# bladesaber/or-tools

Hardware: AMD Instinct MI355X
Metric: simplex iterations/sec + batched LPs/sec, 1/2/4/8 MI355X vs Glop CPU (higher is better)
Workload: dtype f64

## Files before the change

include/mi_lp_devop.h:

```cpp
#ifndef MI_LP_DEVOP_H_
#define MI_LP_DEVOP_H_

#include <stdint.h>

#ifdef __cplusplus
extern "C" {
#endif

typedef struct mi_devop mi_devop;

enum {
  MI_DEVOP_ROW_NONE = 0,
  MI_DEVOP_ROW_SMALL_SERIAL = 1,
  MI_DEVOP_ROW_SMALL_SERIAL_256 = 2,
  MI_DEVOP_ROW_SMALL_BY_COLUMN = 3,
  MI_DEVOP_ROW_MEDIUM_DIRECT = 4,
  MI_DEVOP_ROW_MEDIUM_BATCHED = 5,
  MI_DEVOP_ROW_LIST = 6,
  MI_DEVOP_ROW_FULL_ROWS = 7,
  MI_DEVOP_ROW_CHUNK = 8,
  MI_DEVOP_ROW_BY_COLUMN = 9,
  MI_DEVOP_ROW_COLUMN_WISE_SMALL = 10,
  MI_DEVOP_ROW_COLUMN_WISE_GENERAL = 11
};
enum { MI_DEVOP_COMPACT_NONE = 0, MI_DEVOP_COMPACT_SMALL = 1, MI_DEVOP_COMPACT_CHIP_WIDE = 2 };
enum { MI_DEVOP_RATIO_NONE = 0, MI_DEVOP_RATIO_ONE_WORKGROUP = 1, MI_DEVOP_RATIO_TWO_KERNELS = 2 };

typedef struct mi_devop_paths {
  int32_t update_row;
  int32_t compact;
  int32_t ratio;
  int32_t ratio_tightened;
  int32_t list_mapped;
} mi_devop_paths;

typedef struct mi_devop_api {
  mi_devop* (*create)(int device, int m, int n, const int64_t* col_starts,
                      const int32_t* row_idx, const double* vals);
  void (*destroy)(mi_devop* h);
  const char* (*last_error)(const mi_devop* h);
  int (*set_mask)(mi_devop* h, int which, const uint64_t* words, int num_words);
// ... 6 lines not shown
  int (*read_coefficient)(mi_devop* h, int col, double* out);
  int (*download_coefficients)(mi_devop* h, double* out);
  int (*list_dots_over_update_row)(mi_devop* h, const double* v, double* out, int* count);
  int (*list_dots)(mi_devop* h, const int32_t* cols, int n, const double* v, double* out);
  int (*dual_begin)(mi_devop* h, const double* rc, const uint8_t* colbits,
                    const double* bound_diff);
  int (*dual_set_col_bits)(mi_devop* h, const int32_t* cols, const uint8_t* bits, int n);
  int (*dual_ratio_candidates)(mi_devop* h, double sign, double threshold,
                               double harris_tolerance, double minimum_delta,
                               double variation_magnitude, int32_t* col, double* coeff,
                               double* rc, int* count, int* list_count);
  int (*dual_update_reduced_costs)(mi_devop* h, double mult, int leaving_col,
                                   double leaving_value, int entering_col);
  int (*dual_download_reduced_costs)(mi_devop* h, double* rc);
  int (*last_paths)(mi_devop* h, mi_devop_paths* out);
} mi_devop_api;

extern const mi_devop_api mi_devop_table;

#ifdef __cplusplus
}
#endif

#endif
```

or-tools_amd/csrc/engine/device_lp.h:

```cpp
#ifndef MILP_DEVICE_LP_H_
#define MILP_DEVICE_LP_H_

#include <cstdint>
#include <memory>
#include <mutex>
#include <stdexcept>
#include <string>
#include <vector>

#include "../../../include/mi_lp.h"
#include "device_solver.h"

namespace milp_kernels {
struct TriSolveArgs;
struct ScanState;
struct ListOut;
struct TightenState;
}
namespace sdual {
struct Mailbox;
}

namespace milp {
void SdualProfileReset();
// ... 117 lines not shown
    std::vector<int> runs;
    int chain_levels = 0;
    int max_wide_run = 0;
    int level0_end = 0;
  };
  struct TriContext {
    void* stream = nullptr;
    TriBuffer x, y, top;
    double* h_x = nullptr;
    double* m_x = nullptr;
    size_t h_x_elems = 0;
    int* h_top = nullptr;
    void* graph_exec[kTriNumMatrices] = {};
    uint64_t graph_key[kTriNumMatrices] = {};
    void* ev[2] = {nullptr, nullptr};
  };
  bool TransposeLowerSolve(const TriangularMatrix& t, uint64_t key,
                           std::vector<double>* x) override;
  bool LowerSolve(const TriangularMatrix& lower, uint64_t key,
                  std::vector<double>* x) override;
  bool Solve(TriKind kind, const TriangularMatrix& t, uint64_t key, int start,
             std::vector<double>* x) override;
  bool SolvePair(TriKind kind, const TriangularMatrix& t, uint64_t key, std::vector<double>* x0,
                 std::vector<double>* x1) override;
  bool StartAsyncU(const TriangularMatrix& t, uint64_t key, const std::vector<double>& x) override;
  void FinishAsyncU(std::vector<double>* x) override;
  void DropAsyncU() override;
  bool SpecFlipEnabled() const { return spec_flip_ && tri_mapped_ && !tri_graph_; }

  void SetTiming(bool on, uint32_t id_mask = ~0u);
  bool Timed(int id) const { return timing_ && (timing_ids_ >> (id & 31) & 1u) != 0; }
// ... 118 lines not shown
  void LaunchColumnDots(int mode, const double* d_y, const double* d_c, double* d_out,
                        const double* d_y2 = nullptr, double* d_out2 = nullptr);
  void Check(int err, const char* what);
  void BuildTriSchedule(TriSchedule* s, int nc, int fni, bool ones, const double* diag,
                        const int64_t* st, const int32_t* idx, const double* val, bool reverse,
                        bool descending, bool sequential, uint64_t key, void* stream);
  bool TriSolve(int which, const TriangularMatrix& t, uint64_t key, std::vector<double>* x);
  bool TriPrepare(int which, const TriangularMatrix& t, uint64_t key, int slot,
                  const std::vector<double>& x);
  void TransposeColumns(const TriangularMatrix& t, bool descending);
  void TriReserve(TriBuffer* b, size_t bytes);
  void PrepareTriContext(int slot, int rows, int pos);
  milp_kernels::TriSolveArgs TriArgs(const TriSchedule& s, const TriContext& c) const;
  void TriCopyIn(const TriSchedule& s, const TriContext& c);
  void TriCopyOut(const TriSchedule& s, const TriContext& c);
  void EnqueueTriKernels(const TriSchedule& s, const milp_kernels::TriSolveArgs& a,
                         void* stream);
  void CaptureTriGraph(int which, TriContext* c);
  void FreeTriBuffers();

  void* sdual_arena_ = nullptr;
  void* sdual_staging_ = nullptr;
  void* sdual_staging_dev_ = nullptr;
  size_t sdual_cap_ = 0;
  void* sdual_mb_block_ = nullptr;
  size_t sdual_mb_cap_ = 0;
  sdual::Mailbox* sdual_mb_ = nullptr;
  int32_t* sdual_mb_basis_ = nullptr;
  char* sdual_mb_image_ = nullptr;
  void* sdual_mb_device_ = nullptr;

  int device_ = -1;
// ... 184 lines not shown
  unsigned long long* d_keys_in_ = nullptr;
  unsigned long long* d_keys_out_ = nullptr;
  int32_t* d_sorted_slots_ = nullptr;
  void* d_sort_temp_ = nullptr;
  size_t sort_temp_bytes_ = 0;
  int tri_mode_ = 0;
  int tri_min_rows_ = 16384;
  int tri_wide_level_ = 600;
  int tri_debug_left_ = 0;
  bool tri_graph_ = false;
  bool tri_tau_ = true;
  bool tri_mapped_ = true;
  bool tri_syncfree_ = true;
  int tri_syncfree_min_levels_ = 0;
  bool tri_fuse0_ = true;
  int tri_poll_max_ = 1;
  int tri_persist_groups_ = 0;
  int tri_xcd_stride_ = 1;
  bool stream_priority_ = false;
  bool stream_priority_env_ = false;
  bool stream_prioritized_ = false;
  void SetStreamPriority(bool high);
  bool tri_lower_ = true;
  bool tri_btran_ = false;
  bool tri_pair_ = true;
  bool tri_pad_ = false;
  int tri_min_width_ = 128;
  bool tri_chain_ = false;
  int tri_chain_width_ = 512;
  int tri_chain_min_levels_ = 4;
// ... 11 lines not shown
    int cap_n = 0, cap_t = 0;
  };
  DenseTail dense_tail_;
  int dense_tail_mode_ = 0;
  int64_t dense_tail_min_entries_ = int64_t{1} << 20;
  int dense_tail_min_cols_ = 128;
  bool DenseTailSolve(const TriangularMatrix& t, uint64_t key, std::vector<double>* x);
  void FreeDenseTail();
  TriSchedule tri_sched_[kTriNumMatrices];
  static constexpr int kTriSlots = 4;
  TriContext tri_ctx_[kTriSlots];
  struct AsyncU {
    bool active = false;
    bool trivial = false;
    bool timed = false;
    int rows = 0;
    int first = 0;
    int top = 0;
    double bytes = 0.0;
  };
  AsyncU async_u_;
  bool spec_flip_ = true;
  std::mutex tri_mu_;
  void* h_tri_stage_ = nullptr;
  size_t tri_stage_bytes_ = 0;
  std::vector<int64_t> tri_lt_starts_;
  std::vector<int32_t> tri_lt_idx_;
  std::vector<double> tri_lt_val_;
};

// ... 4 lines not shown
```

or-tools_amd/csrc/engine/device_lp.hip:

```cpp
#include "device_lp.h"
#include "fibers.h"
#include "host_pool.h"

#include <algorithm>
#include <hip/hip_runtime.h>

#include <atomic>
#include <limits>
#include <chrono>
#include <condition_variable>
#include <mutex>
#include <thread>
#include <rocprim/device/device_radix_sort.hpp>

#include <chrono>
#include <cstdlib>
#include <cstring>

#include "lp_data.h"

#include "../kernels/kernel_args.h"

namespace milp {

// ... 153 lines not shown
    dense_tail_min_entries_ = std::atoll(v);
  }
  if (const char* v = std::getenv("MILP_DENSE_TAIL_MIN_COLS")) {
    dense_tail_min_cols_ = std::max(1, std::atoi(v));
  }
  if (const char* v = std::getenv("MILP_TRI_MIN_WIDTH")) tri_min_width_ = std::atoi(v);
  if (const char* v = std::getenv("MILP_TRI_CHAIN")) tri_chain_ = std::atoi(v) != 0;
  if (const char* v = std::getenv("MILP_TRI_CHAIN_WIDTH")) tri_chain_width_ = std::atoi(v);
  if (const char* v = std::getenv("MILP_TRI_CHAIN_MIN_LEVELS")) {
    tri_chain_min_levels_ = std::max(1, std::atoi(v));
  }
  if (const char* v = std::getenv("MILP_TRI_SYNCFREE_MIN_LEVELS")) {
    tri_syncfree_min_levels_ = std::atoi(v);
  }
  if (const char* v = std::getenv("MILP_TRI_FUSE0")) tri_fuse0_ = std::atoi(v) != 0;
  if (const char* v = std::getenv("MILP_TRI_POLL_MAX")) tri_poll_max_ = std::max(1, std::atoi(v));
  if (const char* v = std::getenv("MILP_TRI_PERSIST")) {
    tri_persist_groups_ = std::max(0, std::min(256, std::atoi(v)));
  }
  if (const char* v = std::getenv("MILP_TRI_XCD")) tri_xcd_stride_ = std::atoi(v) != 0 ? 8 : 1;
  if (const char* v = std::getenv("MILP_SMALL_BATCH")) small_batch_ = std::atoi(v) != 0;
  CreateShards();
  StartWatchdog();
}

template <typename T>
T* DeviceLp::Alloc(size_t n) {
  void* p = nullptr;
  Check(hipMalloc(&p, std::max<size_t>(1, n) * sizeof(T)), "hipMalloc");
  allocations_.push_back(p);
// ... 1679 lines not shown
```

or-tools_amd/csrc/engine/device_probe.cc:

```cpp
#include <cstring>
#include <exception>
#include <string>
#include <vector>

#include "../../../include/mi_lp_devop.h"
#include "device_lp.h"
#include "lp_data.h"

struct mi_devop {
  milp::CompactSparseMatrix csc;
  milp::CompactSparseMatrix csr;
  milp::DeviceLp dev;
  std::vector<uint64_t> relevant;
  std::string error;
};

namespace {

thread_local std::string g_create_error;

template <typename Fn>
int Guard(mi_devop* h, Fn fn) {
  try {
    fn();
    return 0;
  } catch (const std::exception& e) {
    h->error = e.what();
  } catch (...) {
// ... 169 lines not shown
    if (!v.empty()) std::memcpy(rc, v.data(), v.size() * sizeof(double));
  });
}

int LastPaths(mi_devop* h, mi_devop_paths* out) {
  return Guard(h, [&] {
    const milp::DeviceLp::LastPaths p = h->dev.last_paths();
    out->update_row = p.update_row;
    out->compact = p.compact;
    out->ratio = p.ratio;
    out->ratio_tightened = p.ratio_tightened ? 1 : 0;
    out->list_mapped = p.list_mapped ? 1 : 0;
  });
}

static_assert(int{MI_DEVOP_ROW_COLUMN_WISE_GENERAL} == int{milp::DeviceLp::kRowColumnWiseGeneral} &&
                  int{MI_DEVOP_ROW_LIST} == int{milp::DeviceLp::kRowList} &&
                  int{MI_DEVOP_COMPACT_CHIP_WIDE} == int{milp::DeviceLp::kCompactChipWide} &&
                  int{MI_DEVOP_RATIO_TWO_KERNELS} == int{milp::DeviceLp::kRatioTwoKernels},
              "mi_lp_devop.h restates DeviceLp's path enums");

}

extern "C" const mi_devop_api mi_devop_table = {
    Create,           Destroy,
    LastError,        SetMask,
    SetListMirror,    SetSmallBatch,
    UpdateRowRowWise, UpdateRowColumnWise,
    FetchUpdateRow,   ReadCoefficient,
    DownloadCoefficients, ListDotsOverUpdateRow,
    ListDots,         DualBegin,
    DualSetColBits,   DualRatioCandidates,
    DualUpdateReducedCosts, DualDownloadReducedCosts,
    LastPaths,
};
```

or-tools_amd/csrc/engine/device_solve.hip:

```cpp
#include <hip/hip_runtime.h>

#include <algorithm>
#include <atomic>
#include <chrono>
#include <cstdio>
#include <cstdlib>
#include <cstring>
#include <mutex>

#include "../kernels/kernel_args.h"
#include "device_lp.h"
#include "host_pool.h"
#include "lu.h"

namespace milp {

namespace {
inline hipStream_t Stream(void* p) { return reinterpret_cast<hipStream_t>(p); }

struct SolveCallTimer {
  mi_lp_kernel_stats* stats;
  int id;
  std::chrono::steady_clock::time_point t0 = std::chrono::steady_clock::now();
  SolveCallTimer(mi_lp_kernel_stats* s, int i) : stats(s), id(i) {}
// ... 23 lines not shown
  FreeDenseTail();
  for (TriSchedule& s : tri_sched_) {
    for (TriBuffer& b : s.buf) FreeBuffer(&b);
    s = TriSchedule();
  }
  if (d_tri_clock_ != nullptr) (void)hipFree(d_tri_clock_);
  d_tri_clock_ = nullptr;
  DropAsyncU();
  for (int slot = 0; slot < kTriSlots; ++slot) {
    TriContext& c = tri_ctx_[slot];
    for (void* g : c.graph_exec) {
      if (g != nullptr) (void)hipGraphExecDestroy(reinterpret_cast<hipGraphExec_t>(g));
    }
    FreeBuffer(&c.x);
    FreeBuffer(&c.y);
    FreeBuffer(&c.top);
    if (c.h_x != nullptr) (void)hipHostFree(c.h_x);
    if (c.h_top != nullptr) (void)hipHostFree(c.h_top);
    for (void* e : c.ev) {
      if (e != nullptr) (void)hipEventDestroy(reinterpret_cast<hipEvent_t>(e));
    }
    if ((slot == 1 || slot == 3) && c.stream != nullptr) {
      (void)hipStreamSynchronize(Stream(c.stream));
      (void)hipStreamDestroy(Stream(c.stream));
    }
    c = TriContext();
  }
  if (h_tri_stage_ != nullptr) (void)hipHostFree(h_tri_stage_);
  h_tri_stage_ = nullptr;
  tri_stage_bytes_ = 0;
// ... 354 lines not shown
        "H2D");
  Check(hipMemcpyAsync(c.top.ptr, c.h_top, sizeof(int), hipMemcpyHostToDevice, Stream(c.stream)),
        "H2D");
}

void DeviceLp::TriCopyOut(const TriSchedule& s, const TriContext& c) {
  if (tri_mapped_) return;
  const int fni = s.first_col;
  const size_t in = size_t(s.rows - fni);
  const double* d_x = static_cast<const double*>(c.x.ptr);
  Check(hipMemcpyAsync(c.h_x + fni, d_x + fni, in * sizeof(double), hipMemcpyDeviceToHost,
                       Stream(c.stream)),
        "D2H");
}

void DeviceLp::EnqueueTriKernels(const TriSchedule& s, const milp_kernels::TriSolveArgs& a,
                                 void* stream) {
  if (tri_persist_groups_ > 0 && tri_syncfree_ && a.clock == nullptr &&
      s.levels >= tri_syncfree_min_levels_) {
    Check(milp_launch::tri_transpose_lower_persistent(a, tri_persist_groups_, tri_xcd_stride_,
                                                      Stream(stream)),
          "tri persistent");
    return;
  }
  if (tri_syncfree_ && a.clock == nullptr && s.max_wide_run <= milp_kernels::kTriSyncFreeMaxWork &&
      s.levels >= tri_syncfree_min_levels_) {
    Check(milp_launch::tri_transpose_lower_syncfree(a, s.runs.data(),
                                                    static_cast<int>(s.runs.size() / 3),
                                                    Stream(stream)),
          "tri syncfree");
    return;
  }
  Check(milp_launch::tri_transpose_lower(a, s.segments.data(),
                                         static_cast<int>(s.segments.size() / 2),
                                         Stream(stream)),
        "tri_transpose_lower");
}

void DeviceLp::CaptureTriGraph(int which, TriContext* c) {
  if (c->graph_exec[which] != nullptr) {
    (void)hipGraphExecDestroy(reinterpret_cast<hipGraphExec_t>(c->graph_exec[which]));
    c->graph_exec[which] = nullptr;
  }
  const TriSchedule& s = tri_sched_[which];
  hipGraph_t graph = nullptr;
  Check(hipStreamBeginCapture(Stream(c->stream), hipStreamCaptureModeThreadLocal), "capture");
  EnqueueTriKernels(s, TriArgs(s, *c), c->stream);
  Check(hipStreamEndCapture(Stream(c->stream), &graph), "capture end");
  hipGraphExec_t exec = nullptr;
  const hipError_t e = hipGraphInstantiate(&exec, graph, nullptr, nullptr, 0);
  (void)hipGraphDestroy(graph);
// ... 270 lines not shown
                     s.chain_levels);
      }
    }
    if (!s.ok) return false;
    if (tri_mode_ == 0 && s.work < int64_t(s.levels - s.chain_levels) * tri_min_width_) {
      return false;
    }
    PrepareTriContext(slot, nc, s.pos);
  }
  return true;
}

bool DeviceLp::TriSolve(int which, const TriangularMatrix& t, uint64_t key,
                        std::vector<double>* x) {
  const int slot = g_lu_slot == 0 ? 0 : 1;
  if (slot != 0 && !tri_tau_) return false;
  const TriKind kind = static_cast<TriKind>(which);
  const int id = slot != 0                       ? MI_K_TRI_SOLVE_TAU
                 : kind == TriKind::kUpperT      ? MI_K_TRI_SOLVE
                 : kind == TriKind::kLower       ? MI_K_TRI_SOLVE_L
                 : kind == TriKind::kUpper       ? MI_K_TRI_SOLVE_UPPER
                                                 : MI_K_TRI_SOLVE_T;
  SolveCallTimer timer(&stats_, id);
  DeviceOp(which == kTriU ? (slot == 0 ? "tri U enter" : "tri U enter (slot 1)")
                          : (slot == 0 ? "tri L enter" : "tri L enter (slot 1)"));
  if (!TriPrepare(which, t, key, slot, *x)) return false;
  const int nc = t.num_cols();
  TriContext& c = tri_ctx_[slot];
  TriSchedule& s = tri_sched_[which];
  double* xv = x->data();
  const int fni = s.first_col;
  int top = nc - 1;
  if (kind == TriKind::kUpperT || kind == TriKind::kLowerT) {
    while (top >= fni && xv[top] == 0.0) --top;
    if (top < fni) return true;
  }
  if (s.rows_upto[top + 1] - s.rows_upto[fni] == 0) return true;
  const size_t in = size_t(nc - fni);
  FtranTimer ft(kFtDevCopyIn);
  CopyHost(c.h_x + fni, xv + fni, in * sizeof(double));
  ft.Lap(kFtDevRun);
  *c.h_top = top;
  int* h_words = reinterpret_cast<int*>(c.h_x + nc);
  h_words[0] = top;
  h_words[1] = 0;
  const double rows = s.rows_upto[top + 1] - s.rows_upto[fni];
  const double entries = static_cast<double>(s.entries_upto[top + 1] - s.entries_upto[fni]);
  const double bytes = rows * (24.0 + (s.ones ? 0.0 : 8.0)) + entries * 20.0 +
                       double(s.pos) * 20.0 + rows * 20.0;
  if (slot == 0 && which == kTriU && tri_debug_left_ > 0) {
    milp_kernels::TriSolveArgs a = TriArgs(s, c);
    if (d_tri_clock_ == nullptr) {
      Check(hipMalloc(reinterpret_cast<void**>(&d_tri_clock_), 65536 * sizeof(uint64_t)),
            "hipMalloc");
    }
    Check(hipMemsetAsync(d_tri_clock_, 0, 65536 * sizeof(uint64_t), Stream(c.stream)),
          "memset");
    if (s.levels + 1 < 65536) a.clock = d_tri_clock_;
    TriCopyIn(s, c);
    BeginKernel(id);
    EnqueueTriKernels(s, a, c.stream);
    EndKernel(id, bytes);
    TriCopyOut(s, c);
    g_overlap.Run();
    Synchronize();
    --tri_debug_left_;
    std::vector<uint64_t> clk(s.levels + 1);
    Check(hipMemcpy(clk.data(), d_tri_clock_, clk.size() * sizeof(uint64_t),
                    hipMemcpyDeviceToHost),
          "D2H");
    const TriSchedule& l = tri_sched_[kTriL];
    std::fprintf(stderr,
                 "[tri] U: rows %d work %d levels %d segments %zu top %d entries/row max %d "
                 ">4 %d >16 %d >64 %d | L: work %d levels %d entries/row max %d >4 %d >16 %d "
                 ">64 %d; U per level (us/width):",
                 nc, s.work, s.levels, s.segments.size() / 2, top, s.max_entries,
// ... 11 lines not shown
      std::lock_guard<std::mutex> lock(tri_mu_);
      CaptureTriGraph(which, &c);
      DeviceOp("tri capture done");
    }
    TriCopyIn(s, c);
    if (slot == 0) {
      BeginKernel(id);
    } else if (Timed(id)) {
      Check(hipEventRecord(reinterpret_cast<hipEvent_t>(c.ev[0]), Stream(c.stream)), "ev");
    }
    if (tri_graph_) {
      Check(hipGraphLaunch(reinterpret_cast<hipGraphExec_t>(c.graph_exec[which]),
                           Stream(c.stream)),
            "graph launch");
    } else {
      EnqueueTriKernels(s, TriArgs(s, c), c.stream);
    }
    if (slot == 0) {
      EndKernel(id, bytes);
    } else if (Timed(id)) {
      Check(hipEventRecord(reinterpret_cast<hipEvent_t>(c.ev[1]), Stream(c.stream)), "ev");
    }
    TriCopyOut(s, c);
    if (slot == 0) g_overlap.Run();
    DeviceOp("tri sync");
    Check(hipStreamSynchronize(Stream(c.stream)), "sync");
    DeviceOp("tri sync done");
    if (slot != 0) {
      stats_.launches[id] += 1;
      stats_.algorithmic_bytes[id] += bytes;
      if (Timed(id)) {
// ... 4 lines not shown
        stats_.device_ms[id] += ms;
      }
    }
  }
  if (*static_cast<volatile int*>(h_words + 1) != 0) {
    throw DeviceError("triangular solve: dependency wait timed out");
  }
  ft.Lap(kFtDevCopyOut);
  CopyHost(xv + fni, c.h_x + fni, size_t(top - fni + 1) * sizeof(double));
  return true;
}

bool DeviceLp::SolvePair(TriKind kind, const TriangularMatrix& t, uint64_t key,
                         std::vector<double>* x0, std::vector<double>* x1) {
  if (kind != TriKind::kUpperT || !tri_pair_ || g_lu_slot != 0) return false;
  if (!tri_syncfree_ || !tri_mapped_ || tri_graph_ || tri_persist_groups_ > 0) return false;
  if (tri_debug_left_ > 0) return false;
  SolveCallTimer timer(&stats_, MI_K_TRI_SOLVE);
  DeviceOp("tri U pair enter");
  if (!TriPrepare(kTriU, t, key, 0, *x0)) return false;
  if (static_cast<int>(x1->size()) < t.num_cols()) return false;
  TriSchedule& s = tri_sched_[kTriU];
  if (s.max_wide_run > milp_kernels::kTriSyncFreeMaxWork || s.levels < tri_syncfree_min_levels_) {
    return false;
  }
  const int nc = t.num_cols();
  const int fni = s.first_col;
  {
    std::lock_guard<std::mutex> lock(tri_mu_);
    PrepareTriContext(2, nc, s.pos);
  }
  TriContext& c0 = tri_ctx_[0];
  TriContext& c1 = tri_ctx_[2];
  std::vector<double>* xs[2] = {x0, x1};
  TriContext* cs[2] = {&c0, &c1};
  int tops[2];
  double bytes = 0.0;
  for (int v = 0; v < 2; ++v) {
    const double* xv = xs[v]->data();
    int top = nc - 1;
    while (top >= fni && xv[top] == 0.0) --top;
    if (top < fni || s.rows_upto[top + 1] - s.rows_upto[fni] == 0) return false;
    tops[v] = top;
    const double rows = s.rows_upto[top + 1] - s.rows_upto[fni];
    const double entries = static_cast<double>(s.entries_upto[top + 1] - s.entries_upto[fni]);
    bytes += rows * (24.0 + (s.ones ? 0.0 : 8.0)) + entries * 20.0 + double(s.pos) * 20.0 +
             rows * 20.0;
  }
  const size_t in = size_t(nc - fni);
  for (int v = 0; v < 2; ++v) {
    TriContext& c = *cs[v];
    CopyHost(c.h_x + fni, xs[v]->data() + fni, in * sizeof(double));
    int* words = reinterpret_cast<int*>(c.h_x + nc);
    words[0] = tops[v];
    words[1] = 0;
  }
  milp_kernels::TriSolveArgs a = TriArgs(s, c0);
  a.x2 = static_cast<double*>(c1.x.ptr);
  a.y2 = static_cast<double*>(c1.y.ptr);
  a.host_x2 = c1.m_x;
  a.top2 = static_cast<int*>(c1.top.ptr);
  a.fail2 = reinterpret_cast<int*>(c1.m_x + s.rows) + 1;
  BeginKernel(MI_K_TRI_SOLVE);
  Check(milp_launch::tri_transpose_lower_syncfree(a, s.runs.data(),
                                                  static_cast<int>(s.runs.size() / 3),
                                                  Stream(c0.stream), 2),
        "tri pair");
  EndKernel(MI_K_TRI_SOLVE, bytes);
  g_overlap.Run();
  DeviceOp("tri pair sync");
  Check(hipStreamSynchronize(Stream(c0.stream)), "sync");
  for (int v = 0; v < 2; ++v) {
    const int* words = reinterpret_cast<const int*>(cs[v]->h_x + nc);
    if (*static_cast<const volatile int*>(words + 1) != 0) {
      throw DeviceError("triangular solve: dependency wait timed out");
    }
  }
  for (int v = 0; v < 2; ++v) {
    CopyHost(xs[v]->data() + fni, cs[v]->h_x + fni, size_t(tops[v] - fni + 1) * sizeof(double));
  }
  return true;
}

bool DeviceLp::StartAsyncU(const TriangularMatrix& t, uint64_t key, const std::vector<double>& x) {
  if (g_lu_slot != 0 || !spec_flip_ || !tri_mapped_ || tri_graph_ || tri_debug_left_ > 0) {
    return false;
  }
  DropAsyncU();
  if (!TriPrepare(kTriU, t, key, 3, x)) return false;
  const int nc = t.num_cols();
  TriContext& c = tri_ctx_[3];
  TriSchedule& s = tri_sched_[kTriU];
  const int fni = s.first_col;
  int top = nc - 1;
  while (top >= fni && x[top] == 0.0) --top;
  async_u_.active = true;
  async_u_.trivial = top < fni || s.rows_upto[top + 1] - s.rows_upto[fni] == 0;
  if (async_u_.trivial) return true;
  DeviceOp("tri U async enter");
  CopyHost(c.h_x + fni, x.data() + fni, size_t(nc - fni) * sizeof(double));
  int* h_words = reinterpret_cast<int*>(c.h_x + nc);
  h_words[0] = top;
  h_words[1] = 0;
  const double rows = s.rows_upto[top + 1] - s.rows_upto[fni];
  const double entries = static_cast<double>(s.entries_upto[top + 1] - s.entries_upto[fni]);
  async_u_.bytes = rows * (24.0 + (s.ones ? 0.0 : 8.0)) + entries * 20.0 +
                   double(s.pos) * 20.0 + rows * 20.0;
  async_u_.rows = nc;
  async_u_.first = fni;
  async_u_.top = top;
  async_u_.timed = Timed(MI_K_TRI_SOLVE);
  if (async_u_.timed) {
    Check(hipEventRecord(reinterpret_cast<hipEvent_t>(c.ev[0]), Stream(c.stream)), "ev");
  }
  EnqueueTriKernels(s, TriArgs(s, c), c.stream);
  if (async_u_.timed) {
    Check(hipEventRecord(reinterpret_cast<hipEvent_t>(c.ev[1]), Stream(c.stream)), "ev");
  }
  return true;
}

void DeviceLp::FinishAsyncU(std::vector<double>* x) {
  if (!async_u_.active) throw DeviceError("asynchronous U solve: none in flight");
  async_u_.active = false;
  if (async_u_.trivial) return;
  TriContext& c = tri_ctx_[3];
  DeviceOp("tri U async sync");
  Check(hipStreamSynchronize(Stream(c.stream)), "sync");
  stats_.launches[MI_K_TRI_SOLVE] += 1;
  stats_.algorithmic_bytes[MI_K_TRI_SOLVE] += async_u_.bytes;
  if (async_u_.timed && Timed(MI_K_TRI_SOLVE)) {
    float ms = 0.0f;
    Check(hipEventElapsedTime(&ms, reinterpret_cast<hipEvent_t>(c.ev[0]),
                              reinterpret_cast<hipEvent_t>(c.ev[1])),
          "ev time");
    stats_.device_ms[MI_K_TRI_SOLVE] += ms;
  }
  const int nc = async_u_.rows;
  if (*reinterpret_cast<volatile int*>(reinterpret_cast<int*>(c.h_x + nc) + 1) != 0) {
    throw DeviceError("triangular solve: dependency wait timed out");
  }
  const int fni = async_u_.first;
  CopyHost(x->data() + fni, c.h_x + fni, size_t(async_u_.top - fni + 1) * sizeof(double));
}

void DeviceLp::DropAsyncU() {
  if (!async_u_.active) return;
  async_u_.active = false;
  if (!async_u_.trivial && tri_ctx_[3].stream != nullptr) {
    (void)hipStreamSynchronize(Stream(tri_ctx_[3].stream));
  }
}

}
```

or-tools_amd/csrc/kernels/kernel_args.h:

```cpp
#ifndef MILP_KERNEL_ARGS_H_
#define MILP_KERNEL_ARGS_H_

#include <hip/hip_runtime.h>
#include <stdint.h>

namespace milp_kernels {

struct DotArgs {
  const int64_t* starts;
  const int32_t* rows;
  const double* vals;
  const double* y;
  int ncols;
  const int32_t* col_list;
  const uint64_t* mask;
  const double* c;
  double* out;
  uint8_t* flags;
  double drop_tolerance;
  const uint8_t* skip;
  const double* y2;
  double* out2;
};

// ... 252 lines not shown
  int seg_begin;
  int seg_end;
  int level0_end;
};
__host__ __device__ inline TriSolveArgs TriRhs(const TriSolveArgs& a, int rhs) {
  TriSolveArgs b = a;
  if (rhs == 1) {
    b.x = a.x2;
    b.y = a.y2;
    b.host_x = a.host_x2;
    b.top = a.top2;
    b.fail = a.fail2;
  }
  return b;
}
constexpr int kTriSyncFreeMaxWork = 512 * 256;
constexpr int kTriChainVals = 12288;

constexpr int kTailMaxCols = 16384;
struct DenseTailArgs {
  const int64_t* starts;
  const int32_t* rows;
  const double* vals;
  const double* diag;
  double* x;
  double* pre;
  int64_t* cur;
  const double* host_x;
  double* host_out;
  int n;
// ... 54 lines not shown
                                int max_count, double mult, int leaving_col,
                                double leaving_value, int entering_col, double* rc,
                                hipStream_t s);
hipError_t set_double(double* dst, double value, hipStream_t s);
hipError_t set_colbits(const int32_t* cols, const uint8_t* bits, int n, uint8_t* colbits,
                       hipStream_t s);
hipError_t set_mask_words(const int32_t* idx, const uint64_t* words, int n, uint64_t* mask,
                          hipStream_t s);
hipError_t boxed_flips(const int32_t* cols, int n, const double* rc, const uint8_t* colbits,
                       double threshold, uint8_t* flag, hipStream_t s);
hipError_t tri_transpose_lower(const milp_kernels::TriSolveArgs& args, const int* segments,
                               int num_segments, hipStream_t s);
hipError_t tri_transpose_lower_syncfree(const milp_kernels::TriSolveArgs& args,
                                        const int* segs, int num_segs, hipStream_t s,
                                        int num_rhs = 1);
hipError_t tri_transpose_lower_persistent(const milp_kernels::TriSolveArgs& args, int groups,
                                          int xcd_stride, hipStream_t s);
hipError_t column_squared_norms(const int64_t* starts, const double* vals,
                                const uint64_t* relevant, int ncols, double* out,
                                hipStream_t s);
hipError_t dense_tail_upper_solve(const milp_kernels::DenseTailArgs& args, hipStream_t s);

}

#endif
```

or-tools_amd/csrc/kernels/tri_solve.hip:

```cpp
#include <hip/hip_runtime.h>

#include "kernel_args.h"

namespace milp_kernels {

__device__ __forceinline__ double load_final(const double* y, int k) {
  return __hip_atomic_load(y + k, __ATOMIC_RELAXED, __HIP_MEMORY_SCOPE_AGENT);
}

struct TriRec {
  int row;
  int n;
  int4 e;
  double v[4];
  double d;
};

__device__ __forceinline__ void tri_load(const TriSolveArgs& a, int k, int le, int top,
                                         TriRec* r) {
  const bool in = k < le;
  const int kk = in ? k : 0;
  r->row = in ? a.rec_row[kk] : top + 1;
  r->n = a.rec_n[kk];
  r->e = a.rec_entry[kk];
// ... 324 lines not shown
    if (y1 != 0.0) sum -= y1 * r.v[1];
    if (y2 != 0.0) sum -= y2 * r.v[2];
    if (y3 != 0.0) sum -= y3 * r.v[3];
    return tri_sequential_divide(a, sum, r.d);
  }
  if (n == 4) {
    sum -= r.v[0] * y0 + r.v[1] * y1 + r.v[2] * y2 + r.v[3] * y3;
  } else {
    if (n > 0) sum -= r.v[0] * y0;
    if (n > 1) sum -= r.v[1] * y1;
    if (n > 2) sum -= r.v[2] * y2;
  }
  return a.diag != nullptr ? sum / r.d : sum;
}

__device__ __forceinline__ void tri_syncfree_output(const TriSolveArgs& a, int k, int top) {
  TriRec r;
  tri_load(a, k, a.num_work, top, &r);
  bool done = r.row > top;
  double* y = a.y;
  const double in = done ? 0.0 : a.x[r.row];
  int backoff = 1;
  const uint64_t t0 = wall_clock64();
  const double pend = __longlong_as_double(static_cast<long long>(kTriPending));
  const int n = r.n;
  double y0 = n > 0 ? pend : 0.0, y1 = n > 1 ? pend : 0.0;
  double y2 = n > 2 ? pend : 0.0, y3 = n > 3 ? pend : 0.0;
  double sum = in;
  int e = r.e.x;
  const int end = r.e.x + r.n;
  uint64_t t_progress = t0;
  while (__ballot(!done) != 0) {
    if (done) continue;
    if (n <= 4) {
      if (tri_pending(y0)) y0 = load_final(y, r.e.x);
      if (tri_pending(y1)) y1 = load_final(y, r.e.y);
// ... 69 lines not shown
      t_progress = wall_clock64();
      backoff = 1;
    } else if (wall_clock64() - t_progress > kTriMaxWaitTicks) {
      if (a.fail != nullptr) __hip_atomic_store(a.fail, 1, __ATOMIC_RELAXED, __HIP_MEMORY_SCOPE_SYSTEM);
      done = true;
    } else {
      tri_backoff(a, &backoff);
    }
  }
}

__global__ __launch_bounds__(256) void tri_syncfree_kernel(TriSolveArgs a0) {
  const TriSolveArgs a = TriRhs(a0, blockIdx.y);
  const int k = a.seg_begin + blockIdx.x * blockDim.x + threadIdx.x;
  if (k >= a.seg_end) return;
  tri_syncfree_output(a, k, *a.top);
}

__global__ __launch_bounds__(kTriThreads) void tri_syncfree_persistent_kernel(TriSolveArgs a,
                                                                              int xcd_stride) {
  if (blockIdx.x % xcd_stride != 0) return;
  const int group = blockIdx.x / xcd_stride;
  const int total = (gridDim.x / xcd_stride) * kTriThreads;
  const int top = *a.top;
  for (int k = group * kTriThreads + threadIdx.x; k < a.num_work; k += total) {
    if (k >= a.level0_end) tri_syncfree_output(a, k, top);
  }
}

__device__ __forceinline__ double tri_chain_load(const TriSolveArgs& a, const double* vals,
                                                 const int* ready, int p) {
  if (p >= a.seg_begin && p < a.seg_end) {
    if (__hip_atomic_load(ready + (p - a.seg_begin), __ATOMIC_ACQUIRE,
                          __HIP_MEMORY_SCOPE_WORKGROUP) == 0) {
      return __longlong_as_double(static_cast<long long>(kTriPending));
    }
    return vals[p - a.seg_begin];
  }
  return load_final(a.y, p);
}

// ... 195 lines not shown
    if (a.seg_end <= a.seg_begin) continue;
    if (segs[3 * i + 2] != 0) {
      milp_kernels::tri_chain_kernel<<<dim3(1, num_rhs), milp_kernels::kTriThreads, 0, s>>>(a);
    } else {
      milp_kernels::tri_syncfree_kernel<<<dim3((a.seg_end - a.seg_begin + 255) / 256, num_rhs),
                                          256, 0, s>>>(a);
    }
    e = hipGetLastError();
    if (e != hipSuccess) return e;
  }
  if (args.host_x == nullptr) return hipSuccess;
  milp_kernels::tri_copy_out_kernel<<<dim3(row_blocks, num_rhs), 256, 0, s>>>(args);
  return hipGetLastError();
}

hipError_t tri_transpose_lower_persistent(const milp_kernels::TriSolveArgs& args, int groups,
                                          int xcd_stride, hipStream_t s) {
  if (args.num_work <= 0) return hipSuccess;
  const int row_blocks =
      std::max(1, std::min(1024, (args.num_rows - args.first_col + 255) / 256));
  hipError_t e;
  if (args.host_x != nullptr) {
    milp_kernels::tri_copy_in_kernel<<<row_blocks, 256, 0, s>>>(args);
    e = hipGetLastError();
    if (e != hipSuccess) return e;
  }
  const int pos_blocks = std::max(1, std::min(1024, (args.num_pos + 255) / 256));
  milp_kernels::tri_init_kernel<<<pos_blocks, 256, 0, s>>>(args);
  e = hipGetLastError();
  if (e != hipSuccess) return e;
// ... 52 lines not shown
```

Baseline: 1021.

## Fuse triangular solve init and sync-free pass with double-buffered pending arrays

Adds a fused path for the transposed upper triangular solve. It drops the separate init kernel by keeping two pending-filled y buffers that alternate between calls, and the fused kernel re-arms the idle buffer while it solves. Level-0 outputs are written directly inside the sync-free kernel instead of in a separate pass. This cuts one kernel launch and one full pending fill per solve. In exchange it needs buffer state tracking that must be invalidated on failures and key changes. It also adds probe API entries and plan reporting.

```diff
diff --git a/include/mi_lp_devop.h b/include/mi_lp_devop.h
--- a/include/mi_lp_devop.h
+++ b/include/mi_lp_devop.h
@@ -25,6 +25,20 @@
 };
 enum { MI_DEVOP_COMPACT_NONE = 0, MI_DEVOP_COMPACT_SMALL = 1, MI_DEVOP_COMPACT_CHIP_WIDE = 2 };
 enum { MI_DEVOP_RATIO_NONE = 0, MI_DEVOP_RATIO_ONE_WORKGROUP = 1, MI_DEVOP_RATIO_TWO_KERNELS = 2 };
+
+enum {
+  MI_DEVOP_TRI_NONE = 0,
+  MI_DEVOP_TRI_FUSED = 1,
+  MI_DEVOP_TRI_SYNC_FREE = 2,
+  MI_DEVOP_TRI_PERSISTENT = 3,
+  MI_DEVOP_TRI_LEVELS = 4
+};
+enum {
+  MI_DEVOP_TRI_SYNC = 0,
+  MI_DEVOP_TRI_ASYNC = 1,
+  MI_DEVOP_TRI_ASYNC_START = 2,
+  MI_DEVOP_TRI_ASYNC_DROP = 3
+};
 
 typedef struct mi_devop_paths {
   int32_t update_row;
@@ -61,6 +75,11 @@
                                    double leaving_value, int entering_col);
   int (*dual_download_reduced_costs)(mi_devop* h, double* rc);
   int (*last_paths)(mi_devop* h, mi_devop_paths* out);
+  int (*tri_load)(mi_devop* h, int n, int first_identity, const int64_t* col_starts,
+                  const int32_t* row_idx, const double* vals, const double* diag);
+  int (*tri_solve_u)(mi_devop* h, double* x, double* x1, int async);
+  int (*tri_solve_u_host)(mi_devop* h, double* x);
+  int (*tri_last_plan)(mi_devop* h, int* plan);
 } mi_devop_api;
 
 extern const mi_devop_api mi_devop_table;
diff --git a/or-tools_amd/csrc/engine/device_lp.h b/or-tools_amd/csrc/engine/device_lp.h
--- a/or-tools_amd/csrc/engine/device_lp.h
+++ b/or-tools_amd/csrc/engine/device_lp.h
@@ -155,7 +155,19 @@
     void* graph_exec[kTriNumMatrices] = {};
     uint64_t graph_key[kTriNumMatrices] = {};
     void* ev[2] = {nullptr, nullptr};
-  };
+    TriBuffer fy[2];
+    int fy_next = 0;
+    bool fy_armed = false;
+    uint64_t fy_key = 0;
+  };
+  enum TriPlan {
+    kTriPlanNone = 0,
+    kTriPlanFused = 1,
+    kTriPlanSyncFree = 2,
+    kTriPlanPersistent = 3,
+    kTriPlanLevels = 4,
+  };
+  int tri_last_plan() const { return tri_last_plan_; }
   bool TransposeLowerSolve(const TriangularMatrix& t, uint64_t key,
                            std::vector<double>* x) override;
   bool LowerSolve(const TriangularMatrix& lower, uint64_t key,
@@ -304,8 +316,14 @@
   milp_kernels::TriSolveArgs TriArgs(const TriSchedule& s, const TriContext& c) const;
   void TriCopyIn(const TriSchedule& s, const TriContext& c);
   void TriCopyOut(const TriSchedule& s, const TriContext& c);
-  void EnqueueTriKernels(const TriSchedule& s, const milp_kernels::TriSolveArgs& a,
-                         void* stream);
+  int EnqueueTriKernels(const TriSchedule& s, const milp_kernels::TriSolveArgs& a, void* stream);
+  bool TriFusedApplies(const TriSchedule& s) const;
+  void TriFusedStageIn(const TriSchedule& s, const TriContext& c, const double* x, int top);
+  void TriFusedStageOut(const TriSchedule& s, const TriContext& c, double* x, int top);
+  void TriFusedArm(const TriSchedule& s, TriContext* c);
+  void TriFusedLaunch(const TriSchedule& s, TriContext* const* cs, const int* tops, int num_rhs);
+  bool TriFusedFailed(const TriSchedule& s, TriContext* c);
+  double TriFusedBytes(const TriSchedule& s, int top) const;
   void CaptureTriGraph(int which, TriContext* c);
   void FreeTriBuffers();
 
@@ -520,6 +538,8 @@
   bool tri_syncfree_ = true;
   int tri_syncfree_min_levels_ = 0;
   bool tri_fuse0_ = true;
+  bool tri_fused_ = true;
+  int tri_last_plan_ = 0;
   int tri_poll_max_ = 1;
   int tri_persist_groups_ = 0;
   int tri_xcd_stride_ = 1;
@@ -561,6 +581,7 @@
     bool active = false;
     bool trivial = false;
     bool timed = false;
+    bool fused = false;
     int rows = 0;
     int first = 0;
     int top = 0;
diff --git a/or-tools_amd/csrc/engine/device_lp.hip b/or-tools_amd/csrc/engine/device_lp.hip
--- a/or-tools_amd/csrc/engine/device_lp.hip
+++ b/or-tools_amd/csrc/engine/device_lp.hip
@@ -191,6 +191,7 @@
     tri_syncfree_min_levels_ = std::atoi(v);
   }
   if (const char* v = std::getenv("MILP_TRI_FUSE0")) tri_fuse0_ = std::atoi(v) != 0;
+  if (const char* v = std::getenv("MILP_TRI_FUSED")) tri_fused_ = std::atoi(v) != 0;
   if (const char* v = std::getenv("MILP_TRI_POLL_MAX")) tri_poll_max_ = std::max(1, std::atoi(v));
   if (const char* v = std::getenv("MILP_TRI_PERSIST")) {
     tri_persist_groups_ = std::max(0, std::min(256, std::atoi(v)));
diff --git a/or-tools_amd/csrc/engine/device_probe.cc b/or-tools_amd/csrc/engine/device_probe.cc
--- a/or-tools_amd/csrc/engine/device_probe.cc
+++ b/or-tools_amd/csrc/engine/device_probe.cc
@@ -6,12 +6,15 @@
 #include "../../../include/mi_lp_devop.h"
 #include "device_lp.h"
 #include "lp_data.h"
+#include "lu.h"
 
 struct mi_devop {
   milp::CompactSparseMatrix csc;
   milp::CompactSparseMatrix csr;
   milp::DeviceLp dev;
   std::vector<uint64_t> relevant;
+  milp::TriangularMatrix tri;
+  uint64_t tri_key = 0;
   std::string error;
 };
 
@@ -211,6 +214,79 @@
   });
 }
 
+int TriLoad(mi_devop* h, int n, int first_identity, const int64_t* col_starts,
+            const int32_t* row_idx, const double* vals, const double* diag) {
+  return Guard(h, [&] {
+    h->dev.DropAsyncU();
+    h->tri_key = 0;
+    h->tri.Reset(n, n);
+    milp::SparseColumn col;
+    for (int c = 0; c < n; ++c) {
+      col.Clear();
+      for (int64_t i = col_starts[c]; i < col_starts[c + 1]; ++i) {
+        if (row_idx[i] <= c || row_idx[i] >= n) throw milp::DeviceError("tri_load: bad row");
+        col.AddEntry(row_idx[i], vals[i]);
+      }
+      h->tri.AddTriangularColumnWithGivenDiagonalEntry(col, c, diag[c]);
+    }
+    if (first_identity < 0 || first_identity > h->tri.GetFirstNonIdentityColumn()) {
+      throw milp::DeviceError("tri_load: columns below first_identity are not identity");
+    }
+    h->tri.first_non_identity_column_ = first_identity;
+    static uint64_t next_key = 0;
+    h->tri_key = ++next_key;
+  });
+}
+
+int TriSolveU(mi_devop* h, double* x, double* x1, int async) {
+  return Guard(h, [&] {
+    if (async == MI_DEVOP_TRI_ASYNC_DROP) {
+      h->dev.DropAsyncU();
+      return;
+    }
+    if (h->tri_key == 0) throw milp::DeviceError("tri_solve_u: no matrix loaded");
+    const int n = h->tri.num_cols();
+    std::vector<double> v(x, x + n);
+    if (async == MI_DEVOP_TRI_SYNC && x1 != nullptr) {
+      std::vector<double> v1(x1, x1 + n);
+      if (!h->dev.SolvePair(milp::TriKind::kUpperT, h->tri, h->tri_key, &v, &v1)) {
+        throw milp::DeviceError("tri_solve_u: the device declined the pair");
+      }
+      std::memcpy(x1, v1.data(), n * sizeof(double));
+    } else if (async == MI_DEVOP_TRI_SYNC) {
+      if (!h->dev.Solve(milp::TriKind::kUpperT, h->tri, h->tri_key, 0, &v)) {
+        throw milp::DeviceError("tri_solve_u: the device declined the solve");
+      }
+    } else {
+      if (!h->dev.StartAsyncU(h->tri, h->tri_key, v)) {
+        throw milp::DeviceError("tri_solve_u: the device declined the asynchronous solve");
+      }
+      if (async == MI_DEVOP_TRI_ASYNC) h->dev.FinishAsyncU(&v);
+    }
+    std::memcpy(x, v.data(), n * sizeof(double));
+  });
+}
+
+int TriSolveUHost(mi_devop* h, double* x) {
+  return Guard(h, [&] {
+    if (h->tri_key == 0) throw milp::DeviceError("tri_solve_u_host: no matrix loaded");
+    const int n = h->tri.num_cols();
+    std::vector<double> v(x, x + n);
+    h->tri.TransposeLowerSolve(&v);
+    std::memcpy(x, v.data(), n * sizeof(double));
+  });
+}
+
+int TriLastPlan(mi_devop* h, int* plan) {
+  return Guard(h, [&] { *plan = h->dev.tri_last_plan(); });
+}
+
+static_assert(int{MI_DEVOP_TRI_FUSED} == int{milp::DeviceLp::kTriPlanFused} &&
+                  int{MI_DEVOP_TRI_SYNC_FREE} == int{milp::DeviceLp::kTriPlanSyncFree} &&
+                  int{MI_DEVOP_TRI_PERSISTENT} == int{milp::DeviceLp::kTriPlanPersistent} &&
+                  int{MI_DEVOP_TRI_LEVELS} == int{milp::DeviceLp::kTriPlanLevels},
+              "mi_lp_devop.h restates DeviceLp's plan enum");
+
 static_assert(int{MI_DEVOP_ROW_COLUMN_WISE_GENERAL} == int{milp::DeviceLp::kRowColumnWiseGeneral} &&
                   int{MI_DEVOP_ROW_LIST} == int{milp::DeviceLp::kRowList} &&
                   int{MI_DEVOP_COMPACT_CHIP_WIDE} == int{milp::DeviceLp::kCompactChipWide} &&
@@ -229,5 +305,7 @@
     ListDots,         DualBegin,
     DualSetColBits,   DualRatioCandidates,
     DualUpdateReducedCosts, DualDownloadReducedCosts,
-    LastPaths,
+    LastPaths,        TriLoad,
+    TriSolveU,        TriSolveUHost,
+    TriLastPlan,
 };
diff --git a/or-tools_amd/csrc/engine/device_solve.hip b/or-tools_amd/csrc/engine/device_solve.hip
--- a/or-tools_amd/csrc/engine/device_solve.hip
+++ b/or-tools_amd/csrc/engine/device_solve.hip
@@ -61,6 +61,8 @@
     }
     FreeBuffer(&c.x);
     FreeBuffer(&c.y);
+    FreeBuffer(&c.fy[0]);
+    FreeBuffer(&c.fy[1]);
     FreeBuffer(&c.top);
     if (c.h_x != nullptr) (void)hipHostFree(c.h_x);
     if (c.h_top != nullptr) (void)hipHostFree(c.h_top);
@@ -445,14 +447,14 @@
         "D2H");
 }
 
-void DeviceLp::EnqueueTriKernels(const TriSchedule& s, const milp_kernels::TriSolveArgs& a,
-                                 void* stream) {
+int DeviceLp::EnqueueTriKernels(const TriSchedule& s, const milp_kernels::TriSolveArgs& a,
+                                void* stream) {
   if (tri_persist_groups_ > 0 && tri_syncfree_ && a.clock == nullptr &&
       s.levels >= tri_syncfree_min_levels_) {
     Check(milp_launch::tri_transpose_lower_persistent(a, tri_persist_groups_, tri_xcd_stride_,
                                                       Stream(stream)),
           "tri persistent");
-    return;
+    return kTriPlanPersistent;
   }
   if (tri_syncfree_ && a.clock == nullptr && s.max_wide_run <= milp_kernels::kTriSyncFreeMaxWork &&
       s.levels >= tri_syncfree_min_levels_) {
@@ -460,12 +462,89 @@
                                                     static_cast<int>(s.runs.size() / 3),
                                                     Stream(stream)),
           "tri syncfree");
-    return;
+    return kTriPlanSyncFree;
   }
   Check(milp_launch::tri_transpose_lower(a, s.segments.data(),
                                          static_cast<int>(s.segments.size() / 2),
                                          Stream(stream)),
         "tri_transpose_lower");
+  return kTriPlanLevels;
+}
+
+bool DeviceLp::TriFusedApplies(const TriSchedule& s) const {
+  return tri_fused_ && tri_syncfree_ && tri_mapped_ && !tri_graph_ && tri_persist_groups_ == 0 &&
+         tri_debug_left_ <= 0 && s.levels >= tri_syncfree_min_levels_ && s.work > 0 &&
+         s.pos == s.work && s.chain_levels == 0 && s.runs.size() == 3 &&
+         s.max_wide_run <= milp_kernels::kTriSyncFreeMaxWork;
+}
+
+void DeviceLp::TriFusedStageIn(const TriSchedule& s, const TriContext& c, const double* x,
+                               int top) {
+  const int fni = s.first_col;
+  CopyHost(c.h_x + fni, x + fni, size_t(s.rows - fni) * sizeof(double));
+  int* words = reinterpret_cast<int*>(c.h_x + s.rows);
+  words[0] = top;
+  words[1] = 0;
+}
+
+void DeviceLp::TriFusedStageOut(const TriSchedule& s, const TriContext& c, double* x, int top) {
+  const int fni = s.first_col;
+  CopyHost(x + fni, c.h_x + fni, size_t(top - fni + 1) * sizeof(double));
+}
+
+void DeviceLp::TriFusedArm(const TriSchedule& s, TriContext* c) {
+  const void* old[2] = {c->fy[0].ptr, c->fy[1].ptr};
+  for (TriBuffer& b : c->fy) TriReserve(&b, size_t(s.pos) * 8);
+  if (c->fy_armed && c->fy_key == s.key && c->fy[0].ptr == old[0] && c->fy[1].ptr == old[1]) {
+    return;
+  }
+  for (TriBuffer& b : c->fy) {
+    Check(milp_launch::tri_fill_pending(static_cast<double*>(b.ptr),
+                                        static_cast<int>(b.bytes / 8), Stream(c->stream)),
+          "tri fill");
+  }
+  c->fy_armed = true;
+  c->fy_key = s.key;
+  c->fy_next = 0;
+}
+
+void DeviceLp::TriFusedLaunch(const TriSchedule& s, TriContext* const* cs, const int* tops,
+                              int num_rhs) {
+  for (int v = 0; v < num_rhs; ++v) TriFusedArm(s, cs[v]);
+  milp_kernels::TriSolveArgs a = TriArgs(s, *cs[0]);
+  milp_kernels::TriFusedArgs f{};
+  a.level0_end = 0;
+  a.host_x = cs[0]->m_x;
+  a.y = static_cast<double*>(cs[0]->fy[cs[0]->fy_next].ptr);
+  f.arm0 = static_cast<double*>(cs[0]->fy[1 - cs[0]->fy_next].ptr);
+  f.top0 = tops[0];
+  if (num_rhs == 2) {
+    a.x2 = static_cast<double*>(cs[1]->x.ptr);
+    a.top2 = static_cast<int*>(cs[1]->top.ptr);
+    a.host_x2 = cs[1]->m_x;
+    a.y2 = static_cast<double*>(cs[1]->fy[cs[1]->fy_next].ptr);
+    a.fail2 = reinterpret_cast<int*>(cs[1]->m_x + s.rows) + 1;
+    f.arm1 = static_cast<double*>(cs[1]->fy[1 - cs[1]->fy_next].ptr);
+    f.top1 = tops[1];
+  }
+  Check(milp_launch::tri_transpose_lower_fused(a, f, Stream(cs[0]->stream), num_rhs),
+        "tri fused");
+  for (int v = 0; v < num_rhs; ++v) cs[v]->fy_next = 1 - cs[v]->fy_next;
+}
+
+bool DeviceLp::TriFusedFailed(const TriSchedule& s, TriContext* c) {
+  const int* words = reinterpret_cast<const int*>(c->h_x + s.rows);
+  if (*static_cast<const volatile int*>(words + 1) == 0) return false;
+  c->fy_armed = false;
+  return true;
+}
+
+double DeviceLp::TriFusedBytes(const TriSchedule& s, int top) const {
+  const double rows = s.rows_upto[top + 1] - s.rows_upto[s.first_col];
+  const double entries =
+      static_cast<double>(s.entries_upto[top + 1] - s.entries_upto[s.first_col]);
+  return rows * (24.0 + (s.ones ? 0.0 : 8.0)) + entries * 20.0 + double(s.pos) * 28.0 +
+         rows * 20.0;
 }
 
 void DeviceLp::CaptureTriGraph(int which, TriContext* c) {
@@ -766,6 +845,7 @@
 bool DeviceLp::TriSolve(int which, const TriangularMatrix& t, uint64_t key,
                         std::vector<double>* x) {
   const int slot = g_lu_slot == 0 ? 0 : 1;
+  if (slot == 0 && which == kTriU) tri_last_plan_ = kTriPlanNone;
   if (slot != 0 && !tri_tau_) return false;
   const TriKind kind = static_cast<TriKind>(which);
   const int id = slot != 0                       ? MI_K_TRI_SOLVE_TAU
@@ -788,6 +868,47 @@
     if (top < fni) return true;
   }
   if (s.rows_upto[top + 1] - s.rows_upto[fni] == 0) return true;
+  if (which == kTriU && TriFusedApplies(s)) {
+    FtranTimer ft(kFtDevCopyIn);
+    TriFusedStageIn(s, c, xv, top);
+    ft.Lap(kFtDevRun);
+    const double bytes = TriFusedBytes(s, top);
+    TriContext* cs[1] = {&c};
+    if (slot == 0) {
+      BeginKernel(id);
+    } else if (Timed(id)) {
+      Check(hipEventRecord(reinterpret_cast<hipEvent_t>(c.ev[0]), Stream(c.stream)), "ev");
+    }
+    TriFusedLaunch(s, cs, &top, 1);
+    if (slot == 0) {
+      EndKernel(id, bytes);
+      tri_last_plan_ = kTriPlanFused;
+      g_overlap.Run();
+    } else if (Timed(id)) {
+      Check(hipEventRecord(reinterpret_cast<hipEvent_t>(c.ev[1]), Stream(c.stream)), "ev");
+    }
+    DeviceOp("tri sync");
+    Check(hipStreamSynchronize(Stream(c.stream)), "sync");
+    DeviceOp("tri sync done");
+    if (slot != 0) {
+      stats_.launches[id] += 1;
+      stats_.algorithmic_bytes[id] += bytes;
+      if (Timed(id)) {
+        float ms = 0.0f;
+        Check(hipEventElapsedTime(&ms, reinterpret_cast<hipEvent_t>(c.ev[0]),
+                                  reinterpret_cast<hipEvent_t>(c.ev[1])),
+              "ev time");
+        stats_.device_ms[id] += ms;
+      }
+    }
+    if (TriFusedFailed(s, &c)) {
+      throw DeviceError("triangular solve: dependency wait timed out");
+    }
+    ft.Lap(kFtDevCopyOut);
+    TriFusedStageOut(s, c, xv, top);
+    return true;
+  }
+  if (which == kTriU) c.fy_armed = false;
   const size_t in = size_t(nc - fni);
   FtranTimer ft(kFtDevCopyIn);
   CopyHost(c.h_x + fni, xv + fni, in * sizeof(double));
@@ -811,7 +932,7 @@
     if (s.levels + 1 < 65536) a.clock = d_tri_clock_;
     TriCopyIn(s, c);
     BeginKernel(id);
-    EnqueueTriKernels(s, a, c.stream);
+    tri_last_plan_ = EnqueueTriKernels(s, a, c.stream);
     EndKernel(id, bytes);
     TriCopyOut(s, c);
     g_overlap.Run();
@@ -853,7 +974,8 @@
                            Stream(c.stream)),
             "graph launch");
     } else {
-      EnqueueTriKernels(s, TriArgs(s, c), c.stream);
+      const int plan = EnqueueTriKernels(s, TriArgs(s, c), c.stream);
+      if (slot == 0 && which == kTriU) tri_last_plan_ = plan;
     }
     if (slot == 0) {
       EndKernel(id, bytes);
@@ -888,6 +1010,7 @@
 bool DeviceLp::SolvePair(TriKind kind, const TriangularMatrix& t, uint64_t key,
                          std::vector<double>* x0, std::vector<double>* x1) {
   if (kind != TriKind::kUpperT || !tri_pair_ || g_lu_slot != 0) return false;
+  tri_last_plan_ = kTriPlanNone;
   if (!tri_syncfree_ || !tri_mapped_ || tri_graph_ || tri_persist_groups_ > 0) return false;
   if (tri_debug_left_ > 0) return false;
   SolveCallTimer timer(&stats_, MI_K_TRI_SOLVE);
@@ -916,11 +1039,31 @@
     while (top >= fni && xv[top] == 0.0) --top;
     if (top < fni || s.rows_upto[top + 1] - s.rows_upto[fni] == 0) return false;
     tops[v] = top;
+    if (TriFusedApplies(s)) {
+      bytes += TriFusedBytes(s, top);
+      continue;
+    }
     const double rows = s.rows_upto[top + 1] - s.rows_upto[fni];
     const double entries = static_cast<double>(s.entries_upto[top + 1] - s.entries_upto[fni]);
     bytes += rows * (24.0 + (s.ones ? 0.0 : 8.0)) + entries * 20.0 + double(s.pos) * 20.0 +
              rows * 20.0;
   }
+  if (TriFusedApplies(s)) {
+    for (int v = 0; v < 2; ++v) TriFusedStageIn(s, *cs[v], xs[v]->data(), tops[v]);
+    BeginKernel(MI_K_TRI_SOLVE);
+    TriFusedLaunch(s, cs, tops, 2);
+    EndKernel(MI_K_TRI_SOLVE, bytes);
+    tri_last_plan_ = kTriPlanFused;
+    g_overlap.Run();
+    DeviceOp("tri pair sync");
+    Check(hipStreamSynchronize(Stream(c0.stream)), "sync");
+    const bool failed0 = TriFusedFailed(s, &c0);
+    const bool failed1 = TriFusedFailed(s, &c1);
+    if (failed0 || failed1) throw DeviceError("triangular solve: dependency wait timed out");
+    for (int v = 0; v < 2; ++v) TriFusedStageOut(s, *cs[v], xs[v]->data(), tops[v]);
+    return true;
+  }
+  c0.fy_armed = c1.fy_armed = false;
   const size_t in = size_t(nc - fni);
   for (int v = 0; v < 2; ++v) {
     TriContext& c = *cs[v];
@@ -941,6 +1084,7 @@
                                                   Stream(c0.stream), 2),
         "tri pair");
   EndKernel(MI_K_TRI_SOLVE, bytes);
+  tri_last_plan_ = kTriPlanSyncFree;
   g_overlap.Run();
   DeviceOp("tri pair sync");
   Check(hipStreamSynchronize(Stream(c0.stream)), "sync");
@@ -961,6 +1105,7 @@
     return false;
   }
   DropAsyncU();
+  tri_last_plan_ = kTriPlanNone;
   if (!TriPrepare(kTriU, t, key, 3, x)) return false;
   const int nc = t.num_cols();
   TriContext& c = tri_ctx_[3];
@@ -972,14 +1117,21 @@
   async_u_.trivial = top < fni || s.rows_upto[top + 1] - s.rows_upto[fni] == 0;
   if (async_u_.trivial) return true;
   DeviceOp("tri U async enter");
-  CopyHost(c.h_x + fni, x.data() + fni, size_t(nc - fni) * sizeof(double));
-  int* h_words = reinterpret_cast<int*>(c.h_x + nc);
-  h_words[0] = top;
-  h_words[1] = 0;
-  const double rows = s.rows_upto[top + 1] - s.rows_upto[fni];
-  const double entries = static_cast<double>(s.entries_upto[top + 1] - s.entries_upto[fni]);
-  async_u_.bytes = rows * (24.0 + (s.ones ? 0.0 : 8.0)) + entries * 20.0 +
-                   double(s.pos) * 20.0 + rows * 20.0;
+  async_u_.fused = TriFusedApplies(s);
+  if (async_u_.fused) {
+    TriFusedStageIn(s, c, x.data(), top);
+    async_u_.bytes = TriFusedBytes(s, top);
+  } else {
+    c.fy_armed = false;
+    CopyHost(c.h_x + fni, x.data() + fni, size_t(nc - fni) * sizeof(double));
+    int* h_words = reinterpret_cast<int*>(c.h_x + nc);
+    h_words[0] = top;
+    h_words[1] = 0;
+    const double rows = s.rows_upto[top + 1] - s.rows_upto[fni];
+    const double entries = static_cast<double>(s.entries_upto[top + 1] - s.entries_upto[fni]);
+    async_u_.bytes = rows * (24.0 + (s.ones ? 0.0 : 8.0)) + entries * 20.0 +
+                     double(s.pos) * 20.0 + rows * 20.0;
+  }
   async_u_.rows = nc;
   async_u_.first = fni;
   async_u_.top = top;
@@ -987,7 +1139,13 @@
   if (async_u_.timed) {
     Check(hipEventRecord(reinterpret_cast<hipEvent_t>(c.ev[0]), Stream(c.stream)), "ev");
   }
-  EnqueueTriKernels(s, TriArgs(s, c), c.stream);
+  if (async_u_.fused) {
+    TriContext* cs[1] = {&c};
+    TriFusedLaunch(s, cs, &top, 1);
+    tri_last_plan_ = kTriPlanFused;
+  } else {
+    tri_last_plan_ = EnqueueTriKernels(s, TriArgs(s, c), c.stream);
+  }
   if (async_u_.timed) {
     Check(hipEventRecord(reinterpret_cast<hipEvent_t>(c.ev[1]), Stream(c.stream)), "ev");
   }
@@ -1012,6 +1170,7 @@
   }
   const int nc = async_u_.rows;
   if (*reinterpret_cast<volatile int*>(reinterpret_cast<int*>(c.h_x + nc) + 1) != 0) {
+    c.fy_armed = false;
     throw DeviceError("triangular solve: dependency wait timed out");
   }
   const int fni = async_u_.first;
@@ -1023,7 +1182,12 @@
   async_u_.active = false;
   if (!async_u_.trivial && tri_ctx_[3].stream != nullptr) {
     (void)hipStreamSynchronize(Stream(tri_ctx_[3].stream));
-  }
-}
-
-}
+    TriContext& c = tri_ctx_[3];
+    if (async_u_.fused && c.h_x != nullptr &&
+        *reinterpret_cast<volatile int*>(reinterpret_cast<int*>(c.h_x + async_u_.rows) + 1) != 0) {
+      c.fy_armed = false;
+    }
+  }
+}
+
+}
diff --git a/or-tools_amd/csrc/kernels/kernel_args.h b/or-tools_amd/csrc/kernels/kernel_args.h
--- a/or-tools_amd/csrc/kernels/kernel_args.h
+++ b/or-tools_amd/csrc/kernels/kernel_args.h
@@ -290,6 +290,12 @@
   }
   return b;
 }
+struct TriFusedArgs {
+  double* arm0;
+  double* arm1;
+  int top0;
+  int top1;
+};
 constexpr int kTriSyncFreeMaxWork = 512 * 256;
 constexpr int kTriChainVals = 12288;
 
@@ -374,6 +380,10 @@
 hipError_t tri_transpose_lower_syncfree(const milp_kernels::TriSolveArgs& args,
                                         const int* segs, int num_segs, hipStream_t s,
                                         int num_rhs = 1);
+hipError_t tri_transpose_lower_fused(const milp_kernels::TriSolveArgs& args,
+                                     const milp_kernels::TriFusedArgs& fused, hipStream_t s,
+                                     int num_rhs = 1);
+hipError_t tri_fill_pending(double* y, int n, hipStream_t s);
 hipError_t tri_transpose_lower_persistent(const milp_kernels::TriSolveArgs& args, int groups,
                                           int xcd_stride, hipStream_t s);
 hipError_t column_squared_norms(const int64_t* starts, const double* vals,
diff --git a/or-tools_amd/csrc/kernels/tri_solve.hip b/or-tools_amd/csrc/kernels/tri_solve.hip
--- a/or-tools_amd/csrc/kernels/tri_solve.hip
+++ b/or-tools_amd/csrc/kernels/tri_solve.hip
@@ -362,12 +362,17 @@
   return a.diag != nullptr ? sum / r.d : sum;
 }
 
+template <bool kInit>
 __device__ __forceinline__ void tri_syncfree_output(const TriSolveArgs& a, int k, int top) {
   TriRec r;
   tri_load(a, k, a.num_work, top, &r);
   bool done = r.row > top;
   double* y = a.y;
-  const double in = done ? 0.0 : a.x[r.row];
+  const bool padding = r.row == INT32_MAX;
+  const double in = (kInit ? padding : done) ? 0.0 : a.x[r.row];
+  if (kInit && done && !padding) {
+    __hip_atomic_store(y + k, in, __ATOMIC_RELAXED, __HIP_MEMORY_SCOPE_AGENT);
+  }
   int backoff = 1;
   const uint64_t t0 = wall_clock64();
   const double pend = __longlong_as_double(static_cast<long long>(kTriPending));
@@ -467,7 +472,25 @@
   const TriSolveArgs a = TriRhs(a0, blockIdx.y);
   const int k = a.seg_begin + blockIdx.x * blockDim.x + threadIdx.x;
   if (k >= a.seg_end) return;
-  tri_syncfree_output(a, k, *a.top);
+  tri_syncfree_output<false>(a, k, *a.top);
+}
+
+__global__ __launch_bounds__(256) void tri_fused_kernel(TriSolveArgs a0, TriFusedArgs f) {
+  const int rhs = blockIdx.y;
+  const TriSolveArgs a = TriRhs(a0, rhs);
+  const int k = blockIdx.x * blockDim.x + threadIdx.x;
+  if (k >= a.num_pos) return;
+  __hip_atomic_store((rhs == 0 ? f.arm0 : f.arm1) + k,
+                     __longlong_as_double(static_cast<long long>(kTriPending)),
+                     __ATOMIC_RELAXED, __HIP_MEMORY_SCOPE_AGENT);
+  tri_syncfree_output<true>(a, k, rhs == 0 ? f.top0 : f.top1);
+}
+
+__global__ __launch_bounds__(256) void tri_fill_pending_kernel(double* y, int n) {
+  const double pending = __longlong_as_double(static_cast<long long>(kTriPending));
+  for (int k = blockIdx.x * blockDim.x + threadIdx.x; k < n; k += gridDim.x * blockDim.x) {
+    __hip_atomic_store(y + k, pending, __ATOMIC_RELAXED, __HIP_MEMORY_SCOPE_AGENT);
+  }
 }
 
 __global__ __launch_bounds__(kTriThreads) void tri_syncfree_persistent_kernel(TriSolveArgs a,
@@ -477,7 +500,7 @@
   const int total = (gridDim.x / xcd_stride) * kTriThreads;
   const int top = *a.top;
   for (int k = group * kTriThreads + threadIdx.x; k < a.num_work; k += total) {
-    if (k >= a.level0_end) tri_syncfree_output(a, k, top);
+    if (k >= a.level0_end) tri_syncfree_output<false>(a, k, top);
   }
 }
 
@@ -703,6 +726,33 @@
   return hipGetLastError();
 }
 
+hipError_t tri_transpose_lower_fused(const milp_kernels::TriSolveArgs& args,
+                                     const milp_kernels::TriFusedArgs& fused, hipStream_t s,
+                                     int num_rhs) {
+  if (args.num_work <= 0) return hipSuccess;
+  if (args.num_pos != args.num_work || args.host_x == nullptr ||
+      args.num_pos > milp_kernels::kTriSyncFreeMaxWork) {
+    return hipErrorInvalidValue;
+  }
+  const int row_blocks =
+      std::max(1, std::min(1024, (args.num_rows - args.first_col + 255) / 256));
+  milp_kernels::tri_copy_in_kernel<<<dim3(row_blocks, num_rhs), 256, 0, s>>>(args);
+  const hipError_t e = hipGetLastError();
+  if (e != hipSuccess) return e;
+  milp_kernels::tri_fused_kernel<<<dim3((args.num_pos + 255) / 256, num_rhs), 256, 0, s>>>(args,
+                                                                                          fused);
+  const hipError_t e2 = hipGetLastError();
+  if (e2 != hipSuccess) return e2;
+  milp_kernels::tri_copy_out_kernel<<<dim3(row_blocks, num_rhs), 256, 0, s>>>(args);
+  return hipGetLastError();
+}
+
+hipError_t tri_fill_pending(double* y, int n, hipStream_t s) {
+  if (n <= 0) return hipSuccess;
+  milp_kernels::tri_fill_pending_kernel<<<std::min(1024, (n + 255) / 256), 256, 0, s>>>(y, n);
+  return hipGetLastError();
+}
+
 hipError_t tri_transpose_lower_persistent(const milp_kernels::TriSolveArgs& args, int groups,
                                           int xcd_stride, hipStream_t s) {
   if (args.num_work <= 0) return hipSuccess;
```

After: 978.2. 4.2% lower.
